# lsp-plugins/lsp-dsp-units

Hardware: AMD Instinct MI355X
Metric: Msamples/sec per GPU (biquad-x8 1024ch; Convolver 65536-tap) + HBM roofline % (higher is better)
Workload: dtype f32; 1 GPU; biquad-x8 cascade (FilterBank::process), 1024 channels x 4096-sample blocks per GPU, FLT_BT_LRX_LOPASS slope 4 per-channel cutoffs, state carried across blocks; channels_per_gpu=1024, block=4096, resident_ring_blocks=16, parallelism=channel-shard x1, no collective, blocks_per_call=1657

## Files before the change

lsp-dsp-units_amd/csrc/biquad.hip:

```cpp
#include "mi_common.h"
#include "ilufs_device.h"

#include <algorithm>
#include <atomic>
#include <cmath>
#include <cstdint>
#include <cstdlib>
#include <type_traits>
#include <vector>

namespace
{
    template <int L>
    struct geom
    {
        static constexpr int W      = 2 * L;
        static constexpr int TAB    = 96 + 2 * L;
        static constexpr int PITCH  = W + 4;
        static constexpr int BLOCK  = 64 * W;
        static constexpr int SG     = 128;
        static_assert(((PITCH / 4) & 1) == 1, "LDS pitch must be an odd number of 16-B slots");
        static_assert((TAB % 16) == 0, "table rows stay 64-B aligned (s_load_dwordx16)");
    };

// ... 308 lines not shown
            const int sa = seg_of(c0), sb = seg_of(c0 + L - 1);
            if (sa == sb)
            {
                #pragma unroll
                for (int j = 0; j < 4; ++j)
                    acc[j] += (sa == j) ? q : 0.0f;
                return;
            }
            #pragma unroll
            for (int k = 0; k < L; ++k)
            {
                const float y = hi ? x[k].y : x[k].x;
                const int sk = seg_of(c0 + k);
                #pragma unroll
                for (int j = 0; j < 4; ++j)
                    acc[j] = (sk == j) ? fmaf(y, y, acc[j]) : acc[j];
            }
        };
        auto add_squares = [&](int base)
        {
            v2f q = splat(0.0f);
            #pragma unroll
            for (int k = 0; k < L; ++k)
                q = pk_fma(x[k], x[k], q);
            add_chunk(q.x, base + t * W, false);
            add_chunk(q.y, base + t * W + L, true);
        };




        if (!CHAIN)
        {
            if (ns <= SG)
                load_state(stage_mem(0), 0, ns, 0, 0);
            if (ns > 0)
            {
                load_pq(tb, ctab);
                load_mats(tb, ctab);
                load_coefs(tb, ctab);
            }
            issue_loads(off);
            if (ns <= SG)
                __syncthreads();
        }
        else
        {
            int lds0 = 0;
            for (int k = 0; k < nst; ++k)
            {
                const int nk = stage_ns(k);
                load_state(stage_mem(k), 0, nk, 0, lds0);
                lds0 += nk;
            }
            load_pq(tb, ctab);
            load_mats(tb, ctab);
            load_coefs(tb, ctab);
            issue_loads(off);
            __syncthreads();
        }

        for (int sp = 0; sp < nsup; ++sp)
        {
            const int par  = sp & 1;
            const int base = sp * SUPER + off;
            const int left = n - sp * SUPER;

            #pragma unroll
            for (int k = 0; k < LPT; ++k)
            {
                const int i = 4 * (k * 64 + t);
                *reinterpret_cast<float4 *>(&sx[i + (i / W) * 4]) = ld[k];
            }
            __builtin_amdgcn_wave_barrier();
            MI_PROBE(1 + 4 * sp);
            if (sp + 1 < nsup)
                issue_loads(base + SUPER);
            #pragma unroll
            for (int k = 0; k < L / 4; ++k)
            {
                const float4 a = *reinterpret_cast<const float4 *>(&sx[t * PITCH + 4 * k]);
                const float4 b = *reinterpret_cast<const float4 *>(&sx[t * PITCH + L + 4 * k]);
                x[4 * k + 0] = v2f{a.x, b.x}; x[4 * k + 1] = v2f{a.y, b.y};
                x[4 * k + 2] = v2f{a.z, b.z}; x[4 * k + 3] = v2f{a.w, b.w};
            }

            const int last   = ((left < SUPER) ? left : SUPER) - 1;
            const int w_last = last / SB;
            const int t_last = (last - w_last * SB) / W;
            const bool save_hi = (last - w_last * SB - t_last * W) >= L;
            const bool saver   = (wv == w_last) && (t == t_last);
            if (!CHAIN)
            {
                for (int s0 = 0; s0 < ns; s0 += SG)
                {
                    const int group = (ns - s0 < SG) ? (ns - s0) : SG;
                    if (ns > SG)
                    {
                        __syncthreads();
                        load_state(stage_mem(0), s0, group, par, 0);
                        __syncthreads();
                    }
                    for (int si = 0; si < group; ++si)
                    {
                        const int snext = (s0 + si + 1 < ns) ? s0 + si + 1 : 0;
                        section(tb, ctab + size_t(snext) * TAB, si, par, saver, save_hi);
                    }
                    if (ns > SG)
                    {
                        __syncthreads();
                        flush_state(stage_mem(0), s0, group, par ^ 1, 0);
                    }
                }
                MI_PROBE(2 + 4 * sp);
                if (SUMSQ)
                    add_squares(base);
                else
                    store_block(orsrc, base);
            }
            else
            {
                struct stage_info { int ns; const float *T; float *out; size_t out_stride; int branch; };
                auto fetch = [&](int k) -> stage_info {
                    stage_info q;
                    q.ns = stage_ns(k);
                    q.T = stage_tab(k);
                    q.out = chain.st[k].out;
                    q.out_stride = chain.st[k].out_stride;
                    q.branch = chain.st[k].branch;
                    return q;
                };
                v2f xs[L];
                int lds0 = 0;
                stage_info cur = fetch(0);
                for (int k = 0; k < nst; ++k)
                {
                    const stage_info nxt = fetch((k + 1 < nst) ? k + 1 : 0);
                    if (cur.branch)
                    {
                        #pragma unroll
                        for (int i = 0; i < L; ++i)
                            xs[i] = x[i];
                    }
                    for (int si = 0; si < cur.ns; ++si)
                        section(tb, (si + 1 < cur.ns) ? cur.T + size_t(si + 1) * TAB : nxt.T, lds0 + si, par, saver, save_hi);
                    lds0 += cur.ns;
                    if (cur.out != nullptr)
                    {
                        const __amdgpu_buffer_rsrc_t dst = __builtin_amdgcn_make_buffer_rsrc(
                            cur.out + size_t(ch) * cur.out_stride, 0, n * 4, BUFFER_DWORD3);
                        store_block(dst, base);
                    }
                    if (cur.branch)
                    {
                        #pragma unroll
                        for (int i = 0; i < L; ++i)
                            x[i] = xs[i];
                    }
                    cur = nxt;
                }
            }
            if (NW > 1)
                __syncthreads();
            MI_PROBE(3 + 4 * sp);
        }
        if (!CHAIN)
        {
            if (ns > 0 && ns <= SG)
            {
                __syncthreads();
                flush_state(stage_mem(0), 0, ns, nsup & 1, 0);
            }
        }
        else
        {
            __syncthreads();
            int lds0 = 0;
            for (int k = 0; k < nst; ++k)
            {
                const int nk = stage_ns(k);
                flush_state(stage_mem(k), 0, nk, nsup & 1, lds0);
                lds0 += nk;
            }
        }
        if (SUMSQ)
        {
            __shared__ float red_rows[ROWS][NW][4];
            float (*const red)[4] = red_rows[slot];
            #pragma unroll
            for (int j = 0; j < 4; ++j)
            {
                float v = acc[j];
                #pragma unroll
                for (int d = 32; d > 0; d >>= 1)
                    v += __shfl_xor(v, d);
                if (lane0)
                    red[wv][j] = v;
            }
            __syncthreads();
            if (tid < 4)
            {
                float v = red[0][tid];
                for (int w = 1; w < NW; ++w)
                    v += red[w][tid];
                if (ROWS > 1 || sums_local)
                    sq.sums[slot * 4 + tid] = v;
                else
                    atomicAdd(&sq.sums[size_t(ch) * 4 + tid], v);
            }
        }
        MI_PROBE(15);
    }

    template <int L, int NW, bool ALIGNED>
    __global__ __launch_bounds__(64 * NW, (NW > 1) ? 2 : 1)
    void biquad_bank_kernel(float *out, const float *in, size_t out_stride, size_t in_stride,
                            int n , const float *__restrict__ tab, float *state,
                            const uint32_t *__restrict__ nsec, int max_sec, int out_reread)
    {
        biquad_body<L, NW, ALIGNED, false>(out, in, out_stride, in_stride, n, tab, state, nsec, max_sec, chain_args(), sumsq_args(), false,
                                           out_reread != 0);
    }

    template <int L, int NW, bool ALIGNED>
    __global__ __launch_bounds__(64 * NW, (NW > 1) ? 2 : 1)
    void biquad_sumsq_kernel(const float *in, size_t in_stride, int n , const float *__restrict__ tab,
                             float *state, const uint32_t *__restrict__ nsec, int max_sec, const sumsq_args sq)
    {
        biquad_body<L, NW, ALIGNED, false, true>(nullptr, in, 0, in_stride, n, tab, state, nsec, max_sec, chain_args(), sq);
    }

    template <int L, int NW, bool ALIGNED>
    __global__ __launch_bounds__(64 * NW, (NW > 1) ? 2 : 1)
    void biquad_sumsq_ilufs_kernel(const float *in, size_t in_stride, int n , const float *__restrict__ tab,
                                   float *state, const uint32_t *__restrict__ nsec, int max_sec, const sumsq_args sq,
                                   const mi_meters::ilufs_epilogue ep)
    {
        biquad_body<L, NW, ALIGNED, false, true>(nullptr, in, 0, in_stride, n, tab, state, nsec, max_sec, chain_args(), sq);
        __shared__ uint32_t s_last;
        __shared__ float s_sum[4];
        __shared__ uint32_t s_cnt[4];
        __shared__ float s_val;
        __shared__ float s_chan[2 * 64 * NW];
        const uint32_t meter = blockIdx.x / ep.channels;
        const mi_meters::ilufs_early<64 * NW> early = mi_meters::ilufs_ask<64 * NW>(meter, ep.block, ep.cfg, ep.channels, ep.st, ep.hist,
                                                                                   ep.size, ep.ms_int);
        const mi_meters::ilufs_piece first = ep.pieces.p[0];
        const bool fill_early = ep.out != nullptr && ep.pieces.count > 0 && first.n > 0;
        if (fill_early)
        {
            const uint32_t row = blockIdx.x - meter * ep.channels;
            const uint32_t share = (((first.n + ep.channels - 1) / ep.channels) + 3u) & ~3u;
            const uint32_t a = (row * share < first.n) ? row * share : first.n, b = (a + share < first.n) ? a + share : first.n;
            if (b > a)
                mi_meters::ilufs_fill<64 * NW>(ep.out + size_t(meter) * ep.out_stride + first.offset + a, b - a, early.me.loudness * ep.gain);
        }
        asm volatile("s_waitcnt vmcnt(0)" ::: "memory");
        __syncthreads();
        if (threadIdx.x == 0)
        {
            const uint32_t before = __hip_atomic_fetch_add(&ep.arrived[meter], 1u, __ATOMIC_RELAXED, __HIP_MEMORY_SCOPE_AGENT);
            s_last = (before + 1 == ep.channels) ? 1u : 0u;
            if (s_last)
                __hip_atomic_store(&ep.arrived[meter], 0u, __ATOMIC_RELAXED, __HIP_MEMORY_SCOPE_AGENT);
        }
        __syncthreads();
        if (!s_last)
            return;
        mi_meters::ilufs_call_body<64 * NW, true>(meter, ep.block, sq.sums, ep.pieces, ep.cfg, ep.channels, ep.out, ep.out_stride,
                                            ep.st, ep.gain, ep.hist, ep.size, ep.ms_int, ep.avg, s_sum, s_cnt, s_val, s_chan, early, fill_early);
    }

    template <int L, int NW, bool ALIGNED, int ROWS = 2>
    __global__ __launch_bounds__(ROWS * 64 * NW, 1)
    void biquad_sumsq_ilufs_pair_kernel(const float *in, size_t in_stride, int n , const float *__restrict__ tab,
                                        float *state, const uint32_t *__restrict__ nsec, int max_sec, const sumsq_args sq,
                                        const mi_meters::ilufs_epilogue ep)
    {
        constexpr int TT = ROWS * 64 * NW;
        static_assert(TT == 128 || TT == mi_meters::VTH, "two or four real waves for the 256 virtual threads");
        __shared__ float s_seg[ROWS * 4];
        __shared__ float s_sum[4];
        __shared__ uint32_t s_cnt[4];
        __shared__ float s_val;
        __shared__ float s_chan[2 * TT];
        const uint32_t meter = blockIdx.x;
        const mi_meters::ilufs_early<TT> early = mi_meters::ilufs_ask<TT>(meter, ep.block, ep.cfg, uint32_t(ROWS), ep.st, ep.hist, ep.size, ep.ms_int);
        sumsq_args local = sq;
        local.sums = s_seg;
        biquad_body<L, NW, ALIGNED, false, true, ROWS>(nullptr, in, 0, in_stride, n, tab, state, nsec, max_sec, chain_args(), local, true);
        __syncthreads();
        mi_meters::ilufs_call_body<TT, false, true>(meter, ep.block, s_seg, ep.pieces, ep.cfg, uint32_t(ROWS), ep.out, ep.out_stride,
                                                    ep.st, ep.gain, ep.hist, ep.size, ep.ms_int, ep.avg, s_sum, s_cnt, s_val, s_chan, early);
    }

    template <int L, int NW, bool ALIGNED>
    __global__ __launch_bounds__(64 * NW, (NW > 1) ? 2 : 1)
    void biquad_chain_kernel(const float *in, size_t in_stride, int n , const chain_args chain)
    {
        biquad_body<L, NW, ALIGNED, true>(nullptr, in, 0, in_stride, n, nullptr, nullptr, nullptr, 0, chain);
    }

#ifdef MI_BIQUAD_PROBE
    #define MI_STREAM_PROBE_BEGIN() unsigned long long pc_[4] = {0, 0, 0, 0}, pt_ = __builtin_readcyclecounter(), pw0_ = wall_clock64(), \
        pw1_ = 0, pw2_ = 0; const unsigned long long pc0_ = pt_; unsigned spins_ = 0
    #define MI_STREAM_PROBE(slot) do { __builtin_amdgcn_sched_barrier(0); const unsigned long long now_ = __builtin_readcyclecounter(); \
        pc_[slot] += now_ - pt_; pt_ = now_; if ((slot) == 1 && pw1_ == 0) pw1_ = wall_clock64(); if ((slot) == 3 && pw2_ == 0) pw2_ = wall_clock64(); \
        __builtin_amdgcn_sched_barrier(0); } while (0)
    #define MI_STREAM_PROBE_SPIN() (++spins_)
    #define MI_STREAM_PROBE_ITER(it) do { if (t == 0 && (it) < 20) g_probe[(size_t(blockIdx.x) * NW + wv) * 32 + 11 + (it)] = \
        (wall_clock64() & 0xffffffffull) | ((__builtin_readcyclecounter() & 0xffffffffull) << 32); } while (0)
    #define MI_STREAM_PROBE_END() do { if (t == 0) { unsigned long long *p_ = g_probe + (size_t(blockIdx.x) * NW + wv) * 32; \
        p_[0] = pw0_; p_[1] = wall_clock64(); p_[2] = __builtin_readcyclecounter() - pc0_; p_[3] = pc_[1]; p_[4] = pc_[2]; p_[5] = pc_[3] + pc_[0]; \
        p_[6] = spins_; p_[7] = pw1_; p_[8] = pw2_; \
        p_[9] = __builtin_amdgcn_s_getreg((31 << 11) | 4); p_[10] = __builtin_amdgcn_s_getreg((31 << 11) | 20); } } while (0)
#else
    #define MI_STREAM_PROBE_BEGIN() do { } while (0)
    #define MI_STREAM_PROBE(slot) do { } while (0)
    #define MI_STREAM_PROBE_SPIN() do { } while (0)
    #define MI_STREAM_PROBE_ITER(it) do { } while (0)
    #define MI_STREAM_PROBE_END() do { } while (0)
#endif
#ifndef MI_STREAM_ROTATE
#define MI_STREAM_ROTATE 1
#endif
    constexpr int STREAM_MAX_BLOCKS = 128;
    constexpr int STREAM_SG         = 32;
    struct stream_args
    {
        int             blocks;
        float          *out[STREAM_MAX_BLOCKS];
        const float    *in[STREAM_MAX_BLOCKS];
    };
    constexpr int STREAM_CHAIN_BLOCKS = 64;
    constexpr int STREAM_CHAIN_PTRS   = 320;
    struct stream_chain_stage
    {
        const float    *tab;
        float          *state;
        const uint32_t *nsec;
        int             max_sec;
        int             slot;
        int             branch;
    };
    struct stream_chain_args
    {
        int                 blocks, stages, outs;
        stream_chain_stage  st[CHAIN_MAX];
        const float        *in[STREAM_CHAIN_BLOCKS];
        float              *out[STREAM_CHAIN_PTRS];
    };
    struct stream_kernargs
    {
        stream_args a;
        size_t out_stride, in_stride;
        int n;
        const float *tab;
        float *state;
        const uint32_t *nsec;
        int max_sec, cap;
    };
    struct stream_chain_kernargs
    {
        stream_chain_args c;
        size_t out_stride, in_stride;
        int n, cap;
    };
    struct stream_cell { float d0, d1; uint32_t seq, pad; };
    constexpr uint32_t F_EXACT = 1, F_FINAL = 2, F_SAVE_HI = 4;
    template <class T> __device__ __forceinline__ T here(T v) { asm volatile("" : "+s"(v)); return v; }
    template <class T> __device__ __forceinline__ T here_v(T v) { asm volatile("" : "+v"(v)); return v; }
    typedef volatile __attribute__((address_space(3))) stream_cell lds_cell;

    template <int NW, bool CHAIN, bool QLDS>
    __device__ __forceinline__
    void biquad_stream_body(const stream_args *pa, const stream_chain_args *pc, size_t out_stride, size_t in_stride,
                            int n , const float *__restrict__ tab, float *state,
                            const uint32_t *__restrict__ nsec, int max_sec, int cap)
    {
        using G = geom<16>;
        constexpr int L = 16, W = G::W, TAB = G::TAB, PITCH = G::PITCH, SB = G::BLOCK;
        constexpr int LPT = W / 4;
        constexpr int TAB_QL = TAB_PQ + 2 * L;
        __shared__ __attribute__((aligned(16))) float sx_all[NW * 64 * PITCH];
        extern __shared__ float4 stream_dyn[];
        stream_cell *const cell = reinterpret_cast<stream_cell *>(stream_dyn);
        const float4 *const sql = stream_dyn + cap * NW;

        const int ch  = int(blockIdx.x);
        const int tid = int(threadIdx.x);
        const int t   = tid & 63;
        const int wv  = __builtin_amdgcn_readfirstlane(tid >> 6);
        const int l16 = t & 15;
        float *const sx = sx_all + wv * 64 * PITCH;
        const bool lane0 = (t == 0), row3 = (t >= 48);
        const int nst = CHAIN ? pc->stages : 1;
        auto stage_ns  = [&](int k) -> int { return CHAIN ? int(pc->st[k].nsec[ch]) : int(nsec[ch]); };
        auto stage_tab = [&](int k) -> const float * {
            return CHAIN ? pc->st[k].tab + size_t(ch) * pc->st[k].max_sec * TAB : tab + size_t(ch) * max_sec * TAB; };
        auto stage_mem = [&](int k) -> float * {
            return CHAIN ? pc->st[k].state + size_t(ch) * pc->st[k].max_sec * 2 : state + size_t(ch) * max_sec * 2; };
        const float *ctab = stage_tab(0);
        const int spb   = (n + SB - 1) / SB;
        const int total = (CHAIN ? pc->blocks : pa->blocks) * spb;
        using kargs = typename std::conditional<CHAIN, stream_chain_kernargs, stream_kernargs>::type;
        typedef const __attribute__((address_space(4))) kargs ckargs;
        ckargs *const ka = (ckargs *)__builtin_amdgcn_kernarg_segment_ptr();
        auto ka_blocks = [](ckargs *q) -> int { if constexpr (CHAIN) return q->c.blocks; else return q->a.blocks; };

        typedef const __attribute__((address_space(4))) float cfloat;
        typedef const __attribute__((address_space(4))) v16f cv16f;
        typedef const __attribute__((address_space(4))) v8f cv8f;
        auto uniform_row = [&](const float *T) -> cfloat * {
            const uint64_t v = reinterpret_cast<uint64_t>(T);
            const uint32_t lo = uint32_t(__builtin_amdgcn_readfirstlane(int(uint32_t(v))));
            const uint32_t hi = uint32_t(__builtin_amdgcn_readfirstlane(int(uint32_t(v >> 32))));
            return reinterpret_cast<cfloat *>((uint64_t(hi) << 32) | lo);
        };
        struct sectab
        {
            v16f pq[L / 8];
            v8f  m0;
            v16f m1;
            float4 cf;
            float  a2;
            float4 ql;
        };
        auto load_pq = [&](sectab &r, const float *T)
        {
            cfloat *U = uniform_row(T);
            #pragma unroll
            for (int j = 0; j < L / 8; ++j)
                r.pq[j] = *reinterpret_cast<cv16f *>(U + TAB_PQ + 16 * j);
        };
        auto load_mats = [&](sectab &r, const float *T, int qi )
        {
            cfloat *U = uniform_row(T);
            r.m0 = *reinterpret_cast<cv8f *>(U + 8);
            r.m1 = *reinterpret_cast<cv16f *>(U + 16);
            r.ql = QLDS ? sql[qi * 16 + l16] : *reinterpret_cast<const float4 *>(T + TAB_QL + 4 * l16);
        };
        auto load_coefs = [&](sectab &r, const float *T)
        {
            cfloat *U = uniform_row(T);
            r.cf = make_float4(U[0], U[1], U[2], U[3]);
            r.a2 = U[4];
        };

        const int k0 = wv / spb, j0 = wv - k0 * spb;
        auto advance = [](int &k, int &j, int spb)
        {
            j += NW;
            while (j >= spb)
            {
                j -= spb;
                ++k;
            }
        };
        const int t16 = 16 * t;

        float4 ld[LPT];
        auto issue_loads = [&](ckargs *q, int k, int j, int tq , bool there = true)
        {
            const float *blk;
            if constexpr (CHAIN) blk = q->c.in[k]; else blk = q->a.in[k];
            const __amdgpu_buffer_rsrc_t src = __builtin_amdgcn_make_buffer_rsrc(
                const_cast<float *>(blk + size_t(uint32_t(ch)) * q->in_stride + j * SB), 0, there ? (q->n - j * SB) * 4 : 0, BUFFER_DWORD3);
            #pragma unroll
            for (int q = 0; q < LPT; ++q)
            {
                const u32x4 v = __builtin_amdgcn_raw_buffer_load_b128(src, tq + 1024 * q, 0, 0);
                ld[q] = make_float4(__uint_as_float(v.x), __uint_as_float(v.y), __uint_as_float(v.z), __uint_as_float(v.w));
            }
        };

        if (wv < total)
            issue_loads(ka, k0, j0, t16);
        if (QLDS)
        {
            const __amdgpu_buffer_rsrc_t none = __builtin_amdgcn_make_buffer_rsrc(state, 0, 0, BUFFER_DWORD3);
            #pragma unroll
            for (int q = 0; q < LPT; ++q)
                store_through(none, 4 * (q * 64 + t), make_float4(0.0f, 0.0f, 0.0f, 0.0f));
        }
        const int ns  = stage_ns(0);
        if (!CHAIN && ns < 0)
            return;
        {
            int lds0 = 0;
            for (int k = 0; k < nst; ++k)
            {
                const int nk = (k == 0) ? ns : stage_ns(k);
                const float *mk = stage_mem(k);
                for (int i = tid; i < nk * NW; i += 64 * NW)
                {
                    const int si = i / NW, w = i - si * NW;
                    stream_cell c = { 0.0f, 0.0f, 0u, 0u };
                    if (w == NW - 1)
                    {
                        const float2 s = reinterpret_cast<const float2 *>(mk)[si];
                        c.d0 = s.x;
                        c.d1 = s.y;
                    }
                    cell[(lds0 + si) * NW + w] = c;
                }
                if (QLDS)
                {
                    const float *tk = stage_tab(k);
                    for (int i = tid; i < nk * 16; i += 64 * NW)
                        stream_dyn[cap * NW + lds0 * 16 + i] = *reinterpret_cast<const float4 *>(tk + size_t(i >> 4) * TAB + TAB_QL + 4 * (i & 15));
                }
                lds0 += nk;
            }
        }
        __syncthreads();

        v2f x[L];
        sectab tb;
        if (CHAIN || ns > 0)
        {
            load_pq(tb, ctab);
            load_mats(tb, ctab, 0);
            load_coefs(tb, ctab);
        }
        MI_STREAM_PROBE_BEGIN();

        int k = k0, j = j0;
        if (wv < total) for (int g = wv; ; )
        {
            MI_STREAM_PROBE(0);
            ckargs *const qa = here(ka);
            const int n_a = qa->n, spb_a = (n_a + SB - 1) / SB, total_a = ka_blocks(qa) * spb_a;
            int t_last = 63;
            uint32_t flags = F_SAVE_HI;
            if (j == spb_a - 1)
            {
                const int last = n_a - j * SB - 1;
                t_last = last / W;
                flags = ((last - t_last * W) >= L) ? F_SAVE_HI : 0u;
                flags |= F_EXACT;
            }
            flags |= (j & 1) ? F_EXACT : 0u;
            flags |= (g == total_a - 1) ? F_FINAL : 0u;
            const int tl = here_v(t);
            const bool scan_out = !(flags & F_EXACT) && tl == 63;
            const bool end_out  = (flags & (F_EXACT | F_FINAL)) && tl == t_last;
            const uint32_t want = uint32_t(g), mine = uint32_t(g + 1);

            #pragma unroll
            for (int q = 0; q < LPT; ++q)
            {
                const int i = 4 * (q * 64 + t);
                float *d = &sx[(i / W) * PITCH + 2 * (i % L) + ((i % W) / L)];
                d[0] = ld[q].x; d[2] = ld[q].y; d[4] = ld[q].z; d[6] = ld[q].w;
            }
            __builtin_amdgcn_wave_barrier();
            MI_STREAM_PROBE(1);
            if (!CHAIN && g + NW < total_a)
            {
                int kn = k, jn = j;
                advance(kn, jn, spb_a);
                issue_loads(qa, kn, jn, here_v(t16));
            }
            #pragma unroll
            for (int q = 0; q < L / 2; ++q)
            {
                const float4 v = *reinterpret_cast<const float4 *>(&sx[t * PITCH + 4 * q]);
                x[2 * q] = v2f{v.x, v.y};
                x[2 * q + 1] = v2f{v.z, v.w};
            }

            auto section = [&](const float *Tnext, int qnext, int ci, auto mem2, int turn)
            {
#if MI_STREAM_ROTATE
                if ((turn & 3) == 0)
                    switch (((turn >> 2) + (here(g) / NW) + (here(ch) >> 8)) & 3)
                    {
                        case 0: __builtin_amdgcn_s_setprio(3); break;
                        case 1: __builtin_amdgcn_s_setprio(2); break;
                        case 2: __builtin_amdgcn_s_setprio(1); break;
                        default: __builtin_amdgcn_s_setprio(0); break;
                    }
#endif
                const int w = here(wv);
                lds_cell *const from = (lds_cell *)&cell[ci * NW + ((w + NW - 1) & (NW - 1))];
                lds_cell *const to   = (lds_cell *)&cell[ci * NW + w];
                uint32_t got = from->seq;
                float c0 = from->d0, c1 = from->d1;

                v2f a0 = splat(0.0f), a1_ = splat(0.0f), b0_ = splat(0.0f), b1_ = splat(0.0f);
                #pragma unroll
                for (int q = 0; q < L; q += 2)
                {
                    const v16f &r = tb.pq[q / 8];
                    const v2f pq0 = v2f{r[(2 * q) % 16], r[(2 * q + 1) % 16]};
                    const v2f pq1 = v2f{r[(2 * q + 2) % 16], r[(2 * q + 3) % 16]};
                    a0  = pk_fma(pq0, splat(x[q].x), a0);      b0_ = pk_fma(pq0, splat(x[q].y), b0_);
                    a1_ = pk_fma(pq1, splat(x[q + 1].x), a1_); b1_ = pk_fma(pq1, splat(x[q + 1].y), b1_);
                }
                const v2f zwA = a0 + a1_, zwB = b0_ + b1_;

                const v2f Pc0 = v2f{tb.m0[0], tb.m0[1]}, Pc1 = v2f{tb.m0[2], tb.m0[3]};
                v2f e = mat_fma(Pc0, Pc1, zwA, zwB);
                asm volatile("" : "+v"(e));
                while (got != want)
                {
                    MI_STREAM_PROBE_SPIN();
                    __builtin_amdgcn_s_sleep(1);
                    got = from->seq;
                    c0 = from->d0;
                    c1 = from->d1;
                }
                const v2f cvec = lane0 ? v2f{c0, c1} : splat(0.0f);
                e = mat_fma(v2f{tb.m0[4], tb.m0[5]}, v2f{tb.m0[6], tb.m0[7]}, cvec, e);

                const v2f zero = splat(0.0f);
                e = mat_fma(v2f{tb.m0[4], tb.m0[5]}, v2f{tb.m0[6], tb.m0[7]}, dpp_zero<DPP_ROW_SHR1>(e), e);
                e = mat_fma(v2f{tb.m1[0], tb.m1[1]}, v2f{tb.m1[2], tb.m1[3]}, dpp_zero<DPP_ROW_SHR2>(e), e);
                e = mat_fma(v2f{tb.m1[4], tb.m1[5]}, v2f{tb.m1[6], tb.m1[7]}, dpp_zero<DPP_ROW_SHR4>(e), e);
                e = mat_fma(v2f{tb.m1[8], tb.m1[9]}, v2f{tb.m1[10], tb.m1[11]}, dpp_zero<DPP_ROW_SHR8>(e), e);
                const v2f QLc0 = v2f{tb.ql.x, tb.ql.y}, QLc1 = v2f{tb.ql.z, tb.ql.w};
                e = mat_fma(QLc0, QLc1, dpp_or<DPP_ROW_BCAST15, 0xa>(zero, e), e);
                {
                    const v2f s  = dpp_or<DPP_ROW_BCAST31, 0xc>(zero, e);
                    const v2f s2 = mat_fma(v2f{tb.m1[12], tb.m1[13]}, v2f{tb.m1[14], tb.m1[15]}, s, zero);
                    e = mat_fma(QLc0, QLc1, row3 ? s2 : s, e);
                }
                if (scan_out)
                {
                    to->d0 = e.x;
                    to->d1 = e.y;
                    to->seq = mine;
                }

                const v2f S  = dpp_or<DPP_WAVE_SHR1, 0xf>(cvec, e);
                const v2f SB2 = mat_fma(Pc0, Pc1, S, zwA);
                v2f d0 = v2f{S.x, SB2.x}, d1 = v2f{S.y, SB2.y};
                __builtin_amdgcn_sched_barrier(0);
                load_pq(tb, Tnext);
                load_mats(tb, Tnext, qnext);
                __builtin_amdgcn_sched_barrier(0);

                const v2f b0 = splat(tb.cf.x), b1 = splat(tb.cf.y), b2 = splat(tb.cf.z), a1 = splat(tb.cf.w), a2 = splat(tb.a2);
                #pragma unroll
                for (int q = 0; q < L; ++q)
                {
                    const v2f xx = x[q];
                    const v2f tq = pk_fma(b1, xx, d1);
                    const v2f u  = b2 * xx;
                    const v2f y  = pk_fma(b0, xx, d0);
                    d0   = pk_fma(a1, y, tq);
                    d1   = pk_fma(a2, y, u);
                    x[q] = y;
                }
                __builtin_amdgcn_sched_barrier(0);
                load_coefs(tb, Tnext);
                if (end_out)
                {
                    const uint32_t f = here(flags);
                    const float s0 = (f & F_SAVE_HI) ? d0.y : d0.x, s1 = (f & F_SAVE_HI) ? d1.y : d1.x;
                    if (f & F_EXACT)
                    {
                        to->d0 = s0;
                        to->d1 = s1;
                        to->seq = mine;
                    }
                    if (f & F_FINAL)
                        *mem2() = make_float2(s0, s1);
                }
            };
            auto store_tile = [&](float *rows)
            {
                ckargs *const q = here(ka);
                const int base = here(j) * SB;
                const __amdgpu_buffer_rsrc_t dst = __builtin_amdgcn_make_buffer_rsrc(rows + size_t(uint32_t(ch)) * q->out_stride + base, 0,
                                                                                     (q->n - base) * 4, BUFFER_DWORD3);
                #pragma unroll
                for (int q = 0; q < L / 2; ++q)
                    *reinterpret_cast<float4 *>(&sx[t * PITCH + 4 * q]) = make_float4(x[2 * q].x, x[2 * q].y, x[2 * q + 1].x, x[2 * q + 1].y);
                __builtin_amdgcn_wave_barrier();
                #pragma unroll
                for (int q = 0; q < LPT; ++q)
                {
                    const int i = 4 * (q * 64 + t);
                    const float *d = &sx[(i / W) * PITCH + 2 * (i % L) + ((i % W) / L)];
                    store_through(dst, i, make_float4(d[0], d[2], d[4], d[6]));
                }
                __builtin_amdgcn_wave_barrier();
            };

            if constexpr (!CHAIN)
            {
                const int nsx = here(ns);
                for (int si = 0; si < nsx; ++si)
                {
                    const int snext = (si + 1 < nsx) ? si + 1 : 0;
                    section(ctab + size_t(snext) * TAB, snext, si, [&]() -> float2 * {
                        ckargs *const q = here(ka);
                        return reinterpret_cast<float2 *>(q->state + size_t(uint32_t(ch)) * uint32_t(q->max_sec) * 2) + si; }, si);
                }
                MI_STREAM_PROBE(2);
                store_tile(here(ka)->a.out[here(k)]);
            }
            else
            {
                struct stage_info { int ns; const float *T; float2 *mem2; int slot, branch; };
                auto fetch = [&](int q) -> stage_info {
                    stage_info v;
                    v.ns = stage_ns(q);
                    v.T = stage_tab(q);
                    v.mem2 = reinterpret_cast<float2 *>(stage_mem(q));
                    v.slot = pc->st[q].slot;
                    v.branch = pc->st[q].branch;
                    return v;
                };
                auto run_stage = [&](auto may_branch, const stage_info &cur, const float *Tn, int lds0, int qn )
                {
                    constexpr bool BR = decltype(may_branch)::value;
                    v2f xs[L];
                    if (BR && cur.branch)
                    {
                        #pragma unroll
                        for (int i = 0; i < L; ++i)
                            xs[i] = x[i];
                    }
                    for (int si = 0; si < cur.ns; ++si)
                        section((si + 1 < cur.ns) ? cur.T + size_t(si + 1) * TAB : Tn, (si + 1 < cur.ns) ? lds0 + si + 1 : qn,
                                lds0 + si, [&]() -> float2 * { return cur.mem2 + si; }, lds0 + si);
                    if (cur.slot >= 0)
                        store_tile(pc->out[k * pc->outs + cur.slot]);
                    if (BR && cur.branch)
                    {
                        #pragma unroll
                        for (int i = 0; i < L; ++i)
                            x[i] = xs[i];
                    }
                };
                int lds0 = 0;
                stage_info cur = fetch(0);
                for (int q = 0; q + 1 < nst; ++q)
                {
                    const stage_info nxt = fetch(q + 1);
                    run_stage(std::true_type(), cur, nxt.T, lds0, lds0 + cur.ns);
                    lds0 += cur.ns;
                    cur = nxt;
                }
                {
                    ckargs *const q = here(ka);
                    const int spb_q = (q->n + SB - 1) / SB;
                    const bool more = g + NW < ka_blocks(q) * spb_q;
                    int kn = k, jn = j;
                    if (more)
                        advance(kn, jn, spb_q);
                    issue_loads(q, kn, jn, here_v(t16), more);
                }
                run_stage(std::false_type(), cur, ctab, lds0, 0);
                MI_STREAM_PROBE(2);
            }
            MI_STREAM_PROBE(3);
            MI_STREAM_PROBE_ITER(g / NW);
            {
                ckargs *const q = here(ka);
                const int spb_q = (q->n + SB - 1) / SB;
                advance(k, j, spb_q);
                g = here(g) + NW;
                if (g >= ka_blocks(q) * spb_q)
                    break;
            }
        }
        MI_STREAM_PROBE_END();
    }

    __device__ unsigned long long g_stream_clock[4];

    template <int NW, bool QLDS>
    __global__ __launch_bounds__(64 * NW, (NW >= 4) ? 4 : 2)
    void biquad_stream_kernel(const stream_args a, size_t out_stride, size_t in_stride, int n ,
                              const float *__restrict__ tab, float *state, const uint32_t *__restrict__ nsec, int max_sec, int cap)
    {
        const bool stamp = blockIdx.x == 0 && threadIdx.x == 0;
        if (stamp)
        {
            g_stream_clock[0] = __builtin_readcyclecounter();
            g_stream_clock[1] = wall_clock64();
        }
        biquad_stream_body<NW, false, QLDS>(&a, nullptr, out_stride, in_stride, n, tab, state, nsec, max_sec, cap);
        if (stamp)
        {
            g_stream_clock[2] = __builtin_readcyclecounter();
            g_stream_clock[3] = wall_clock64();
        }
    }

    template <int NW, bool QLDS>
    __global__ __launch_bounds__(64 * NW, 4)
    void biquad_stream_chain_kernel(const stream_chain_args c, size_t out_stride, size_t in_stride, int n , int cap)
    {
        biquad_stream_body<NW, true, QLDS>(nullptr, &c, out_stride, in_stride, n, nullptr, nullptr, nullptr, 0, cap);
    }

    inline bool stream_qlds(int nw, int cap) { return size_t(nw) * 64 * geom<16>::PITCH * 4 + size_t(cap) * (nw + 16) * 16 <= 40960; }
    inline size_t stream_lds(int nw, int cap, bool qlds) { return size_t(cap) * (nw + (qlds ? 16 : 0)) * 16; }

    __global__ void biquad_tail_kernel(float *out, const float *in, size_t out_stride, size_t in_stride,
                                       size_t start, int count , const float *__restrict__ tab, int tab_row,
                                       float *state, const uint32_t *__restrict__ nsec, int max_sec, uint32_t channels,
                                       const sumsq_args sq)
    {
        const uint32_t ch = blockIdx.x * blockDim.x + threadIdx.x;
        if (ch >= channels)
            return;
        const int ns = int(nsec[ch]);
        if (ns < 0)
            return;
        float xs[16];
        for (int k = 0; k < 16; ++k)
            xs[k] = (k < count) ? in[size_t(ch) * in_stride + start + k] : 0.0f;
        for (int s = 0; s < ns; ++s)
        {
            const float *q = tab + (size_t(ch) * max_sec + s) * tab_row;
            float *st = state + (size_t(ch) * max_sec + s) * 2;
            const float b0 = q[0], b1 = q[1], b2 = q[2], a1 = q[3], a2 = q[4];
            float d0 = st[0], d1 = st[1];
            for (int k = 0; k < count; ++k)
            {
                const float xx = xs[k];
                const float tq = fmaf(b1, xx, d1);
// ... 1097 lines not shown
```

Measured before the change: 609,100 Msamples/s.

## Hoist kernarg and table loads ahead of LDS staging in stream kernel prologue

In the non-chain streaming biquad kernel, the prologue now reads the kernel arguments and the first four input-block pointers directly into scalar registers. It issues the section-table, state and quad-table loads before the first input buffer load, and fills the LDS cells and quad table with one store per thread instead of strided loops. It also computes the starting block index without a division. The goal is to shorten the serial startup latency before the first barrier so that loads overlap. The cost is extra register pressure and the assumption that cap fits within the thread count when staging. Probe macros are extended to record entry and staging timestamps.

```diff
diff --git a/lsp-dsp-units_amd/csrc/biquad.hip b/lsp-dsp-units_amd/csrc/biquad.hip
--- a/lsp-dsp-units_amd/csrc/biquad.hip
+++ b/lsp-dsp-units_amd/csrc/biquad.hip
@@ -634,19 +634,25 @@
     }
 
 #ifdef MI_BIQUAD_PROBE
+    __device__ unsigned long long g_probe_start[4096 * 4];
+    #define MI_STREAM_PROBE_ENTRY() const unsigned long long pe_ = wall_clock64(); unsigned long long ps_ = 0
+    #define MI_STREAM_PROBE_STAGED() do { __builtin_amdgcn_sched_barrier(0); ps_ = wall_clock64(); __builtin_amdgcn_sched_barrier(0); } while (0)
     #define MI_STREAM_PROBE_BEGIN() unsigned long long pc_[4] = {0, 0, 0, 0}, pt_ = __builtin_readcyclecounter(), pw0_ = wall_clock64(), \
-        pw1_ = 0, pw2_ = 0; const unsigned long long pc0_ = pt_; unsigned spins_ = 0
+        pw1_ = 0, pw2_ = 0, pw3_ = 0; const unsigned long long pc0_ = pt_; unsigned spins_ = 0
     #define MI_STREAM_PROBE(slot) do { __builtin_amdgcn_sched_barrier(0); const unsigned long long now_ = __builtin_readcyclecounter(); \
         pc_[slot] += now_ - pt_; pt_ = now_; if ((slot) == 1 && pw1_ == 0) pw1_ = wall_clock64(); if ((slot) == 3 && pw2_ == 0) pw2_ = wall_clock64(); \
-        __builtin_amdgcn_sched_barrier(0); } while (0)
+        if ((slot) == 3) pw3_ = wall_clock64(); __builtin_amdgcn_sched_barrier(0); } while (0)
     #define MI_STREAM_PROBE_SPIN() (++spins_)
     #define MI_STREAM_PROBE_ITER(it) do { if (t == 0 && (it) < 20) g_probe[(size_t(blockIdx.x) * NW + wv) * 32 + 11 + (it)] = \
         (wall_clock64() & 0xffffffffull) | ((__builtin_readcyclecounter() & 0xffffffffull) << 32); } while (0)
     #define MI_STREAM_PROBE_END() do { if (t == 0) { unsigned long long *p_ = g_probe + (size_t(blockIdx.x) * NW + wv) * 32; \
         p_[0] = pw0_; p_[1] = wall_clock64(); p_[2] = __builtin_readcyclecounter() - pc0_; p_[3] = pc_[1]; p_[4] = pc_[2]; p_[5] = pc_[3] + pc_[0]; \
         p_[6] = spins_; p_[7] = pw1_; p_[8] = pw2_; \
-        p_[9] = __builtin_amdgcn_s_getreg((31 << 11) | 4); p_[10] = __builtin_amdgcn_s_getreg((31 << 11) | 20); } } while (0)
+        p_[9] = __builtin_amdgcn_s_getreg((31 << 11) | 4); p_[10] = __builtin_amdgcn_s_getreg((31 << 11) | 20); \
+        unsigned long long *q_ = g_probe_start + (size_t(blockIdx.x) * NW + wv) * 4; q_[0] = pe_; q_[1] = ps_; q_[2] = pw3_; q_[3] = 0; } } while (0)
 #else
+    #define MI_STREAM_PROBE_ENTRY() do { } while (0)
+    #define MI_STREAM_PROBE_STAGED() do { } while (0)
     #define MI_STREAM_PROBE_BEGIN() do { } while (0)
     #define MI_STREAM_PROBE(slot) do { } while (0)
     #define MI_STREAM_PROBE_SPIN() do { } while (0)
@@ -714,6 +720,23 @@
         constexpr int L = 16, W = G::W, TAB = G::TAB, PITCH = G::PITCH, SB = G::BLOCK;
         constexpr int LPT = W / 4;
         constexpr int TAB_QL = TAB_PQ + 2 * L;
+        MI_STREAM_PROBE_ENTRY();
+        using kargs = typename std::conditional<CHAIN, stream_chain_kernargs, stream_kernargs>::type;
+        typedef const __attribute__((address_space(4))) kargs ckargs;
+        ckargs *const ka = (ckargs *)__builtin_amdgcn_kernarg_segment_ptr();
+        auto ka_blocks = [](ckargs *q) -> int { if constexpr (CHAIN) return q->c.blocks; else return q->a.blocks; };
+        const float *first[4] = { nullptr, nullptr, nullptr, nullptr };
+        int blocks_all;
+        if constexpr (!CHAIN)
+        {
+            n = ka->n; in_stride = ka->in_stride; max_sec = ka->max_sec; cap = ka->cap;
+            blocks_all = ka->a.blocks;
+            first[0] = ka->a.in[0]; first[1] = ka->a.in[1]; first[2] = ka->a.in[2]; first[3] = ka->a.in[3];
+            asm volatile("" : "+s"(first[0]), "+s"(first[1]), "+s"(first[2]), "+s"(first[3])
+                            : "s"(blocks_all), "s"(n), "s"(in_stride), "s"(max_sec), "s"(cap));
+        }
+        else
+            blocks_all = pc->blocks;
         __shared__ __attribute__((aligned(16))) float sx_all[NW * 64 * PITCH];
         extern __shared__ float4 stream_dyn[];
         stream_cell *const cell = reinterpret_cast<stream_cell *>(stream_dyn);
@@ -734,12 +757,7 @@
             return CHAIN ? pc->st[k].state + size_t(ch) * pc->st[k].max_sec * 2 : state + size_t(ch) * max_sec * 2; };
         const float *ctab = stage_tab(0);
         const int spb   = (n + SB - 1) / SB;
-        const int total = (CHAIN ? pc->blocks : pa->blocks) * spb;
-        using kargs = typename std::conditional<CHAIN, stream_chain_kernargs, stream_kernargs>::type;
-        typedef const __attribute__((address_space(4))) kargs ckargs;
-        ckargs *const ka = (ckargs *)__builtin_amdgcn_kernarg_segment_ptr();
-        auto ka_blocks = [](ckargs *q) -> int { if constexpr (CHAIN) return q->c.blocks; else return q->a.blocks; };
-
+        const int total = blocks_all * spb;
         typedef const __attribute__((address_space(4))) float cfloat;
         typedef const __attribute__((address_space(4))) v16f cv16f;
         typedef const __attribute__((address_space(4))) v8f cv8f;
@@ -765,11 +783,15 @@
             for (int j = 0; j < L / 8; ++j)
                 r.pq[j] = *reinterpret_cast<cv16f *>(U + TAB_PQ + 16 * j);
         };
-        auto load_mats = [&](sectab &r, const float *T, int qi )
+        auto load_mats_s = [&](sectab &r, const float *T)
         {
             cfloat *U = uniform_row(T);
             r.m0 = *reinterpret_cast<cv8f *>(U + 8);
             r.m1 = *reinterpret_cast<cv16f *>(U + 16);
+        };
+        auto load_mats = [&](sectab &r, const float *T, int qi )
+        {
+            load_mats_s(r, T);
             r.ql = QLDS ? sql[qi * 16 + l16] : *reinterpret_cast<const float4 *>(T + TAB_QL + 4 * l16);
         };
         auto load_coefs = [&](sectab &r, const float *T)
@@ -779,7 +801,22 @@
             r.a2 = U[4];
         };
 
-        const int k0 = wv / spb, j0 = wv - k0 * spb;
+        int k0 = 0, j0 = wv;
+        if constexpr (CHAIN)
+        {
+            k0 = wv / spb;
+            j0 = wv - k0 * spb;
+        }
+        else
+        {
+            #pragma unroll
+            for (int i = 1; i < NW; ++i)
+                if (j0 >= spb)
+                {
+                    j0 -= spb;
+                    ++k0;
+                }
+        }
         auto advance = [](int &k, int &j, int spb)
         {
             j += NW;
@@ -792,21 +829,55 @@
         const int t16 = 16 * t;
 
         float4 ld[LPT];
+        auto issue_rows = [&](const float *blk, size_t stride, int len, int j, int tq , bool there)
+        {
+            const __amdgpu_buffer_rsrc_t src = __builtin_amdgcn_make_buffer_rsrc(
+                const_cast<float *>(blk + size_t(uint32_t(ch)) * stride + j * SB), 0, there ? (len - j * SB) * 4 : 0, BUFFER_DWORD3);
+            #pragma unroll
+            for (int q = 0; q < LPT; ++q)
+            {
+                const u32x4 v = __builtin_amdgcn_raw_buffer_load_b128(src, tq + 1024 * q, 0, 0);
+                ld[q] = make_float4(__uint_as_float(v.x), __uint_as_float(v.y), __uint_as_float(v.z), __uint_as_float(v.w));
+            }
+        };
         auto issue_loads = [&](ckargs *q, int k, int j, int tq , bool there = true)
         {
             const float *blk;
             if constexpr (CHAIN) blk = q->c.in[k]; else blk = q->a.in[k];
-            const __amdgpu_buffer_rsrc_t src = __builtin_amdgcn_make_buffer_rsrc(
-                const_cast<float *>(blk + size_t(uint32_t(ch)) * q->in_stride + j * SB), 0, there ? (q->n - j * SB) * 4 : 0, BUFFER_DWORD3);
+            issue_rows(blk, q->in_stride, q->n, j, tq, there);
+        };
+
+        constexpr bool QREG = QLDS && NW >= 4;
+        sectab tb;
+        float2 mem0 = make_float2(0.0f, 0.0f);
+        float4 qop = make_float4(0.0f, 0.0f, 0.0f, 0.0f);
+        int ns;
+        if constexpr (!CHAIN)
+        {
+            ns = stage_ns(0);
+            const int row = tid / NW;
+            mem0 = reinterpret_cast<const float2 *>(stage_mem(0))[(row < cap) ? row : cap - 1];
+            if (QREG)
+            {
+                const int si = ((tid >> 4) < cap) ? (tid >> 4) : cap - 1;
+                qop = *reinterpret_cast<const float4 *>(ctab + size_t(si) * TAB + TAB_QL + 4 * (tid & 15));
+            }
+            load_pq(tb, ctab);
+            load_mats_s(tb, ctab);
+            if (!QLDS)
+                tb.ql = *reinterpret_cast<const float4 *>(ctab + TAB_QL + 4 * l16);
+            load_coefs(tb, ctab);
+            __builtin_amdgcn_sched_barrier(0);
+        }
+        if constexpr (!CHAIN)
+        {
+            const float *blk = first[0];
             #pragma unroll
-            for (int q = 0; q < LPT; ++q)
-            {
-                const u32x4 v = __builtin_amdgcn_raw_buffer_load_b128(src, tq + 1024 * q, 0, 0);
-                ld[q] = make_float4(__uint_as_float(v.x), __uint_as_float(v.y), __uint_as_float(v.z), __uint_as_float(v.w));
-            }
-        };
-
-        if (wv < total)
+            for (int i = 1; i < NW; ++i)
+                blk = (k0 == i) ? first[i] : blk;
+            issue_rows(blk, in_stride, n, j0, t16, wv < total);
+        }
+        else if (wv < total)
             issue_loads(ka, k0, j0, t16);
         if (QLDS)
         {
@@ -815,10 +886,31 @@
             for (int q = 0; q < LPT; ++q)
                 store_through(none, 4 * (q * 64 + t), make_float4(0.0f, 0.0f, 0.0f, 0.0f));
         }
-        const int ns  = stage_ns(0);
-        if (!CHAIN && ns < 0)
-            return;
-        {
+        if constexpr (!CHAIN)
+        {
+            __builtin_amdgcn_sched_barrier(0);
+            asm volatile("" :: "s"(tb.pq[0]), "s"(tb.pq[1]), "s"(tb.m0), "s"(tb.m1), "s"(tb.cf.x), "s"(tb.cf.y), "s"(tb.cf.z), "s"(tb.cf.w),
+                               "s"(tb.a2));
+            if (ns < 0)
+                return;
+            if (tid < cap * NW)
+            {
+                const bool last = (tid & (NW - 1)) == NW - 1;
+                const stream_cell c = { last ? mem0.x : 0.0f, last ? mem0.y : 0.0f, 0u, 0u };
+                cell[tid] = c;
+            }
+            if (QREG)
+            {
+                if (tid < cap * 16)
+                    stream_dyn[cap * NW + tid] = qop;
+            }
+            else if (QLDS)
+                for (int i = tid; i < cap * 16; i += 64 * NW)
+                    stream_dyn[cap * NW + i] = *reinterpret_cast<const float4 *>(ctab + size_t(i >> 4) * TAB + TAB_QL + 4 * (i & 15));
+        }
+        else
+        {
+            ns = stage_ns(0);
             int lds0 = 0;
             for (int k = 0; k < nst; ++k)
             {
@@ -845,16 +937,18 @@
                 lds0 += nk;
             }
         }
+        MI_STREAM_PROBE_STAGED();
         __syncthreads();
 
         v2f x[L];
-        sectab tb;
-        if (CHAIN || ns > 0)
+        if constexpr (CHAIN)
         {
             load_pq(tb, ctab);
             load_mats(tb, ctab, 0);
             load_coefs(tb, ctab);
         }
+        else if (QLDS)
+            tb.ql = sql[l16];
         MI_STREAM_PROBE_BEGIN();
 
         int k = k0, j = j0;
```

Result: no change. 607,300 Msamples/s, median of 2 (-0.3%).
